# neu-vi/Superpoints_Registration

Hardware: AMD Instinct MI355X
Metric: point-cloud pairs/sec (16 384 pts/cloud) (higher is better)
Workload: dtype f32 (matrix products: range-scaled split-f16x2 MFMA, f32 accumulate; attention weights below 2^-5 of their row sum carried in one f16 plane); 1 GPU; synthetic 16384-pt pairs, full KPConv backbone + superpoint attn + Sinkhorn-SVD pose (3dmatch config, BASELINE configs[1]); streams_per_gpu=1, points_per_cloud=16384, generator=box, point_order=reference, upsample_indices=True, cross_step_overlap=True, streams_inside_a_forward=3: main path, pyramid searches, ResNet shortcut branches

## Files before the change

### include/spr.h

```cpp
#ifndef SPR_H_
#define SPR_H_

#include <stddef.h>
#include <stdint.h>

#ifdef __cplusplus
extern "C" {
#endif

#define SPR_VERSION 6

#define SPR_ACT_NONE 0
#define SPR_ACT_RELU 1
#define SPR_ACT_SIGMOID 2

#define SPR_ORDER_REFERENCE 0
#define SPR_ORDER_CANONICAL 1

#define SPR_SELECT_NEAREST 0
#define SPR_SELECT_INDEX 1

int spr_version(void);
const char* spr_last_error(void);

// ... 38 lines not shown
size_t spr_augment_workspace_bytes(int ns, int nt, int nb, int corr_stride);
int spr_augment_pairs(const float* src_xyz, const int* src_cu, int ns, const float* tgt_xyz, const int* tgt_cu,
                      int nt, const float* pose, int nb, const unsigned char* src_mask,
                      const unsigned char* tgt_mask, const int* corr, int corr_stride, const int* corr_off,
                      const int* corr_count, const float* perturb, const unsigned char* flags, int mode, float scale,
                      int max_pts, uint64_t seed, const uint64_t* pair_key, const float* noise,
                      const unsigned int* keys, float* out_src_xyz, float* out_tgt_xyz, int* out_src_cu,
                      int* out_tgt_cu, float* out_pose, unsigned char* out_src_mask, unsigned char* out_tgt_mask,
                      int* out_src_perm, int* out_tgt_perm, int* out_corr, int* out_corr_count, int* status, void* ws,
                      size_t ws_bytes, void* stream);

size_t spr_kpconv_workspace_bytes(int nq, int ns, int cin, int cout);
size_t spr_kpconv_plan_bytes(int nq);
int spr_kpconv_plan(const int* nbr, int nq, int ns, int nbr_stride, int kmax, int rows_sorted,
                    const int* order, void* plan, size_t plan_bytes, void* stream);
size_t spr_kpconv_wplanes_bytes(int cin, int cout);
int spr_kpconv_prep_weights(const float* weights, int n_kp, int cin, int cout, const float* w_range,
                            int w_range_n, void* wplanes, size_t wplanes_bytes, void* stream);
int spr_kpconv_fwd(const float* q_xyz, int nq, const float* s_xyz, int ns, const int* nbr,
                   int nbr_stride, int kmax, int rows_sorted, const float* x, int cin,
                   const float* weights, int cout, const float* kernel_points, int n_kp,
                   float kp_extent, float* out, int impl, const float* x_range, int x_range_n,
                   const float* w_range, int w_range_n, const void* plan, const void* wplanes,
                   void* ws, size_t ws_bytes, void* stream);

size_t spr_instnorm_workspace_bytes(int max_len_host, int nb, int c);
int spr_instnorm(const float* x, const int* cu, int n, int nb, int max_len_host, int c,
                 float eps, int norm, const float* add, float slope, float* out,
                 float* out_range, int out_range_n, void* ws, size_t ws_bytes, void* stream);
int spr_instnorm_stats(const float* x, const int* cu, int n, int nb, int max_len_host, int c, float eps,
                       float* mean, float* rstd, void* ws, size_t ws_bytes, void* stream);

int spr_block_tail_tile_rows(int ka, int kb, int n_out);
size_t spr_block_tail_tiles_len(int n, int nb, int tile_rows);
int spr_block_tail_tiles(const int* cu, int n, int nb, int tile_rows, int* tiles, void* stream);
size_t spr_block_tail_workspace_bytes(int n, int nb, int kb, int n_out, int tile_rows);
int spr_block_tail(const float* xa, int ka, const float* wa, const float* xb, int kb, const float* wb,
                   const float* add, const int* cu, const int* tiles, int n, int nb, int n_out, float eps,
                   float slope, float* out, const float* xa_range, int xa_range_n, const float* wa_range,
                   int wa_range_n, const float* xb_range, int xb_range_n, const float* wb_range,
                   int wb_range_n, float* out_range, int out_range_n, const float* xa_mean,
                   const float* xa_rstd, float xa_slope, void* ws, size_t ws_bytes, void* stream);

int spr_maxpool_gather(const float* x, int ns, int c, const int* idx, int nq, int idx_stride, int k,
                       const int* order, float* out, float* out_range, int out_range_n, void* stream);
size_t spr_cell_order_workspace_bytes(int n);
int spr_cell_order(const float* xyz, const int* cu, int n, int nb, float cell, int* order, void* ws, size_t ws_bytes,
                   void* stream);

size_t spr_linear_workspace_bytes(void);
int spr_linear(const float* x, int m, int k, const float* w, int n, const float* bias,
               const float* residual, int act, float* out, const float* x_range,
// ... 212 lines not shown
```

### superpoints_registration_amd/_lib.py

```python
import ctypes
import os
import subprocess

_HERE = os.path.dirname(os.path.abspath(__file__))
LIB_PATH = os.environ.get("SPR_HIP_LIB") or os.path.join(_HERE, "libspr_hip.so")

_vp = ctypes.c_void_p
_i = ctypes.c_int
_f = ctypes.c_float
_sz = ctypes.c_size_t
_l = ctypes.c_long
_u64 = ctypes.c_uint64

SIGNATURES = {
    "spr_version": (_i, []),
    "spr_last_error": (ctypes.c_char_p, []),
    "spr_grid_subsample_workspace_bytes": (_sz, [_i, _i]),
    "spr_grid_subsample": (_i, [_vp, _vp, _i, _i, _f, _i, _i, _vp, _vp, _vp, _vp, _sz, _vp]),
    "spr_voxel_downsample_workspace_bytes": (_sz, [_i]),
    "spr_voxel_downsample": (_i, [_vp, _i, ctypes.c_double, _vp, _vp, _vp, _sz, _vp]),
    "spr_radius_neighbors_workspace_bytes": (_sz, [_i, _i, _i]),
    "spr_radius_neighbors": (_i, [_vp, _vp, _i, _vp, _vp, _i, _i, _f, _i, _i, _i, _vp, _vp, _vp, _sz, _vp]),
    "spr_radius_table_bytes": (_sz, [_i, _i]),
    "spr_radius_table_build_workspace_bytes": (_sz, [_i, _i]),
    "spr_radius_table_query_workspace_bytes": (_sz, [_i]),
    "spr_radius_table_slots": (_i, []),
    "spr_radius_table_build": (_i, [_vp, _vp, _i, _i, _f, _vp, _sz, _vp, _sz, _vp]),
    "spr_radius_table_query": (_i, [_vp, _vp, _i, _i, _i, _i, _f, _i, _i, _vp, _vp, _vp, _i, _i, _vp, _sz, _vp]),
    "spr_gt_overlap_workspace_bytes": (_sz, [_i, _i, _i]),
    "spr_gt_overlap": (_i, [_vp, _vp, _i, _vp, _vp, _i, _vp, _i, ctypes.c_double, _vp, _vp, _vp, _vp, _vp, _vp, _vp,
                            _sz, _vp]),
    "spr_philox4x32_host": (_i, [_vp, _vp, _vp]),
    "spr_augment_draw": (_i, [_u64, _vp, _i, _i, _vp, _vp, _vp, _vp, _vp, _i, _vp, _i, _vp, _vp, _vp]),
    "spr_augment_workspace_bytes": (_sz, [_i, _i, _i, _i]),
    "spr_augment_pairs": (_i, [_vp, _vp, _i, _vp, _vp, _i, _vp, _i, _vp, _vp, _vp, _i, _vp, _vp, _vp, _vp, _i, _f, _i,
                               _u64, _vp, _vp, _vp, _vp, _vp, _vp, _vp, _vp, _vp, _vp, _vp, _vp, _vp, _vp, _vp, _vp,
                               _sz, _vp]),
    "spr_kpconv_workspace_bytes": (_sz, [_i, _i, _i, _i]),
    "spr_kpconv_fwd": (_i, [_vp, _i, _vp, _i, _vp, _i, _i, _i, _vp, _i, _vp, _i, _vp, _i, _f, _vp, _i, _vp, _i, _vp,
                            _i, _vp, _vp, _vp, _sz, _vp]),
    "spr_instnorm_workspace_bytes": (_sz, [_i, _i, _i]),
    "spr_instnorm": (_i, [_vp, _vp, _i, _i, _i, _i, _f, _i, _vp, _f, _vp, _vp, _i, _vp, _sz, _vp]),
    "spr_maxpool_gather": (_i, [_vp, _i, _i, _vp, _i, _i, _i, _vp, _vp, _vp, _i, _vp]),
    "spr_linear_workspace_bytes": (_sz, []),
    "spr_linear": (_i, [_vp, _i, _i, _vp, _i, _vp, _vp, _i, _vp, _vp, _i, _vp, _i, _vp, _i, _vp, _vp, _sz, _vp]),
    "spr_range_parts": (_i, []),
    "spr_absmax_multi": (_i, [_vp, _i, _i, _vp, _vp]),
    "spr_absmax": (_i, [_vp, _l, _i, _l, _vp, _vp]),
    "spr_kpconv_plan_bytes": (_sz, [_i]),
    "spr_kpconv_plan": (_i, [_vp, _i, _i, _i, _i, _i, _vp, _vp, _sz, _vp]),
    "spr_kpconv_wplanes_bytes": (_sz, [_i, _i]),
    "spr_kpconv_prep_weights": (_i, [_vp, _i, _i, _i, _vp, _i, _vp, _sz, _vp]),
    "spr_block_tail_tile_rows": (_i, [_i, _i, _i]),
    "spr_block_tail_tiles_len": (_sz, [_i, _i, _i]),
    "spr_block_tail_tiles": (_i, [_vp, _i, _i, _i, _vp, _vp]),
    "spr_block_tail_workspace_bytes": (_sz, [_i, _i, _i, _i, _i]),
    "spr_block_tail": (_i, [_vp, _i, _vp, _vp, _i, _vp, _vp, _vp, _vp, _i, _i, _i, _f, _f, _vp, _vp, _i, _vp, _i,
                            _vp, _i, _vp, _i, _vp, _i, _vp, _vp, _f, _vp, _sz, _vp]),
    "spr_instnorm_stats": (_i, [_vp, _vp, _i, _i, _i, _i, _f, _vp, _vp, _vp, _sz, _vp]),
    "spr_cell_order_workspace_bytes": (_sz, [_i]),
    "spr_cell_order": (_i, [_vp, _vp, _i, _i, _f, _vp, _vp, _sz, _vp]),
    "spr_layernorm_range_count": (_i, [_i]),
    "spr_attn_inproj_prepare": (_i, [_vp, _i, _vp, _vp]),
    "spr_set_gemm_mode": (_i, [_i]),
    "spr_layernorm": (_i, [_vp, _i, _i, _vp, _vp, _f, _vp, _vp, _vp, _vp, _vp, _vp]),
# ... 114 lines not shown
```

### superpoints_registration_amd/csrc/kpconv.hip

```cpp
#include "spr_common.h"

namespace spr {
namespace {

constexpr int kKP = 15;

__global__ __launch_bounds__(256) void k_rowflag(const float* __restrict__ x, const float* __restrict__ s_xyz,
                                                 int ns, int cin, unsigned char* __restrict__ flag,
                                                 float4* __restrict__ sxf, int* __restrict__ tile_ctr) {
  const int wid = (blockIdx.x * blockDim.x + threadIdx.x) >> 6;
  const int lane = threadIdx.x & 63;
  const int c4 = cin >> 2;
  if (blockIdx.x == 0 && threadIdx.x == 0) {
    sxf[ns] = make_float4(-1.0e17f, -1.0e17f, -1.0e17f, __int_as_float(0));
    tile_ctr[0] = 0;
  }
  if ((cin & 3) == 0 && c4 <= 64 && (c4 & (c4 - 1)) == 0) {
    constexpr int kRfSteps = 4;
    const int rpl = 64 / c4;
    const int sub = lane / c4, chunk = lane % c4;
    const int row0 = wid * rpl * kRfSteps + sub;
    float4 v[kRfSteps];
#pragma unroll
    for (int r = 0; r < kRfSteps; ++r) {
// ... 28 lines not shown
      }
    }
    return;
  }
  const int row = wid;
  if (row >= ns) return;
  float s = 0.f;
  for (int c = lane; c < cin; c += 64) s += x[(size_t)row * cin + c];
  s = wave_sum(s);
  if (lane == 0) {
    const int f = s > 0.f ? 1 : 0;
    flag[row] = (unsigned char)f;
    sxf[row] = make_float4(s_xyz[3 * (size_t)row], s_xyz[3 * (size_t)row + 1],
                           s_xyz[3 * (size_t)row + 2], __int_as_float(f));
  }
}

__global__ void k_kpconv_simple(const float* __restrict__ q_xyz, int nq,
                                const float* __restrict__ s_xyz, int ns,
                                const int* __restrict__ nbr, int nbr_stride, int kmax,
                                const float* __restrict__ x, int cin,
                                const float* __restrict__ W, int cout,
                                const float* __restrict__ kpts, int n_kp, float inv_extent,
                                const unsigned char* __restrict__ flag,
                                float* __restrict__ out) {
  const long gid = (long)blockIdx.x * blockDim.x + threadIdx.x;
  if (gid >= (long)nq * cout) return;
  const int n = (int)(gid / cout), o = (int)(gid % cout);
  const float qx = q_xyz[3 * (size_t)n], qy = q_xyz[3 * (size_t)n + 1], qz = q_xyz[3 * (size_t)n + 2];
  float acc = 0.f;
  int cnt = 0;
  for (int k = 0; k < kmax; ++k) {
    const int idx = nbr[(size_t)n * nbr_stride + k];
    if (idx < 0 || idx >= ns) continue;
    cnt += flag[idx];
    const float rx = s_xyz[3 * (size_t)idx] - qx, ry = s_xyz[3 * (size_t)idx + 1] - qy,
                rz = s_xyz[3 * (size_t)idx + 2] - qz;
    for (int p = 0; p < n_kp; ++p) {
      const float dx = rx - kpts[3 * p], dy = ry - kpts[3 * p + 1], dz = rz - kpts[3 * p + 2];
      const float w = fmaxf(0.f, 1.f - sqrtf(dx * dx + dy * dy + dz * dz) * inv_extent);
      if (w > 0.f) {
        float d = 0.f;
        for (int c = 0; c < cin; ++c)
          d += x[(size_t)idx * cin + c] * W[((size_t)p * cin + c) * cout + o];
        acc += w * d;
      }
    }
  }
  out[(size_t)n * cout + o] = acc / (float)max(cnt, 1);
}

__global__ __launch_bounds__(256) void k_records_cin1(const float* __restrict__ x, const float* __restrict__ s_xyz,
                                                      int ns, float4* __restrict__ sxf) {
  const int i = blockIdx.x * blockDim.x + threadIdx.x;
  if (i < ns) sxf[i] = make_float4(s_xyz[3 * (size_t)i], s_xyz[3 * (size_t)i + 1], s_xyz[3 * (size_t)i + 2], x[i]);
}

__global__ __launch_bounds__(256) void k_kpconv_cin1(
// ... 1066 lines not shown
  hipStream_t stream = (hipStream_t)stream_;
  SPR_REQUIRE(n_kp == kKP && cin % 32 == 0 && cout % 32 == 0 && cout <= 256,
              "kpconv weight planes exist for the MFMA shapes only (15 kernel points, channels in multiples of 32)");
  SPR_REQUIRE(w_range != nullptr && w_range_n >= 1, "kpconv weight planes: the weight range is required");
  Workspace w(wplanes, bytes);
  const auto [wh, wl] = wplanes_view(w, cin, cout);
  SPR_REQUIRE(wplanes != nullptr && w.ok(), "kpconv weight planes: buffer too small");
  hipLaunchKernelGGL(k_w_prep, dim3(cdiv((long)n_kp * cin * cout, 256)), dim3(256), 0, stream, weights, cin, cout,
                     w_chunk(cin), w_range, w_range_n, wh, wl);
  SPR_LAUNCH_CHECK();
  return 0;
}

extern "C" size_t spr_kpconv_workspace_bytes(int nq, int ns, int cin, int cout) {
  return measure(kpconv_layout, nq, ns, cin, cout);
}

extern "C" int spr_kpconv_fwd(const float* q_xyz, int nq, const float* s_xyz, int ns,
                              const int* nbr, int nbr_stride, int kmax, int rows_sorted,
                              const float* x, int cin, const float* weights, int cout,
                              const float* kernel_points, int n_kp, float kp_extent,
                              float* out, int impl, const float* x_range, int x_range_n, const float* w_range,
                              int w_range_n, const void* plan, const void* wplanes, void* ws, size_t ws_bytes,
                              void* stream_) {
  hipStream_t stream = (hipStream_t)stream_;
  SPR_REQUIRE((x_range == nullptr || x_range_n >= 1) && (w_range == nullptr || w_range_n >= 1),
              "kpconv: a range needs a count");
  SPR_REQUIRE(nq > 0 && ns > 0, "kpconv: empty input");
  SPR_REQUIRE(kmax >= 1 && kmax <= nbr_stride, "kpconv: bad kmax=%d stride=%d", kmax, nbr_stride);
  SPR_REQUIRE(cin >= 1 && cout >= 1 && n_kp >= 1 && n_kp <= 32, "kpconv: bad dims");
  SPR_REQUIRE(kp_extent > 0.f, "kpconv: KP_extent must be > 0");
  Workspace w(ws, ws_bytes);
  const auto [flag, sxf, own_wplanes, x_parts, w_parts, own_plan, tile_ctr] = kpconv_layout(w, nq, ns, cin, cout);
  SPR_REQUIRE(ws != nullptr && w.ok(), "kpconv: workspace too small");
  SPR_REQUIRE(wplanes == nullptr || w_range != nullptr, "kpconv: prepared weight planes come with the range they were scaled by");
  Workspace given_w(const_cast<void*>(wplanes), SIZE_MAX), given_p(const_cast<void*>(plan), SIZE_MAX);
  const auto [wh, wl] = wplanes != nullptr ? wplanes_view(given_w, cin, cout) : own_wplanes;
  const float inv_extent = 1.0f / kp_extent;

  if (cin == 1 && (impl == 0 || impl == 2) && n_kp <= 16) {
    hipLaunchKernelGGL(k_records_cin1, dim3(cdiv(ns, 256)), dim3(256), 0, stream, x, s_xyz, ns, sxf);
    ProfScope prof(stream, cin * 100000 + cout, nq);
    hipLaunchKernelGGL(k_kpconv_cin1, dim3(cdiv(nq, 64)), dim3(256), 0, stream, q_xyz, nq, s_xyz, ns, nbr,
                       nbr_stride, kmax, rows_sorted, sxf, weights, cout, kernel_points, n_kp, inv_extent, out);
    SPR_LAUNCH_CHECK();
    return 0;
  }

  launch_rowflag(x, s_xyz, ns, cin, flag, sxf, tile_ctr, stream);
  SPR_LAUNCH_CHECK();

  const bool tile_fits = cin % 64 == 0 ? mfma_lds_bytes(64, kTile64TQ, kTileWaves, kmax) <= kMfmaLdsMax
                                       : mfma_lds_bytes(32, kTile32TQ, kTileWaves, kmax) <= kMfmaLdsMax;
  if ((impl == 0 || impl == 2) && n_kp == kKP && cin % 32 == 0 && cout % 32 == 0 && cout <= 256 && tile_fits) {
    const int ktot = n_kp * cin;
    const float* xp = x_range != nullptr ? x_range : x_parts;
    const float* wp = w_range != nullptr ? w_range : w_parts;
    const int n_xp = x_range != nullptr ? x_range_n : kAmaxParts, n_wp = w_range != nullptr ? w_range_n : kAmaxParts;
    if (x_range == nullptr && w_range == nullptr) {
      if (int rc = launch_absmax2(x, ns, cin, cin, x_parts, weights, ktot, cout, cout, w_parts, stream)) return rc;
    } else if (x_range == nullptr) {
      if (int rc = launch_absmax(x, ns, cin, cin, x_parts, stream)) return rc;
    } else if (w_range == nullptr) {
      if (int rc = launch_absmax(weights, ktot, cout, cout, w_parts, stream)) return rc;
    }
    if (wplanes == nullptr)
      hipLaunchKernelGGL(k_w_prep, dim3(cdiv((long)ktot * cout, 256)), dim3(256), 0, stream, weights, cin, cout,
                         w_chunk(cin), wp, n_wp, wh, wl);
    const bool ring_ok = impl == 0 && ring_shape(cin, cout) && kmax <= 128 && (size_t)ns * cin * 4 < (1ull << 32) &&
                         (size_t)nq * nbr_stride * 4 < (1ull << 32);
    if (ring_ok) {
      if (plan == nullptr)
        if (int rc = launch_plan(nbr, nq, ns, nbr_stride, kmax, rows_sorted, nullptr, own_plan, stream)) return rc;
      const auto [desc, pad_word] = plan != nullptr ? plan_view(given_p, nq) : own_plan;
#define SPR_RING_ARGS                                                                                       \
  q_xyz, nq, ns, nbr, nbr_stride, kmax, x, wh, wl, kernel_points, inv_extent, sxf, desc, pad_word, xp, wp, \
      n_xp, n_wp, tile_ctr, out, stream
      if (cin == 64 && cout == 64) return launch_ring<64, 64, SPR_KP_NS64>(SPR_RING_ARGS);
      if (cin == 64 && cout == 32) return launch_ring<64, 32, 4>(SPR_RING_ARGS);
      if (cin == 32 && cout == 32) return launch_ring<32, 32, 3>(SPR_RING_ARGS);
      if (cin == 32 && cout == 64) return launch_ring<32, 64, 8>(SPR_RING_ARGS);
      if (cin == 32 && cout == 128) return launch_ring<32, 128, 8>(SPR_RING_ARGS);
#undef SPR_RING_ARGS
    }
#define SPR_KP_ARGS                                                                         \
  q_xyz, nq, s_xyz, ns, nbr, nbr_stride, kmax, rows_sorted, x, cin, wh, wl, cout,           \
      kernel_points, inv_extent, sxf, xp, wp, n_xp, n_wp, out, stream
    if (cin % 64 == 0) {
      if (cout == 64) return launch_mfma<64, kTile64TQ, 1, kTileWaves, 2>(SPR_KP_ARGS);
      if (cout == 128) return launch_mfma<64, kTile64TQ, 2, kTileWaves, 2>(SPR_KP_ARGS);
      if (cout == 256) return launch_mfma<64, kTile64TQ, 4, kTileWaves, 2>(SPR_KP_ARGS);
    } else {
      if (cout == 32) return launch_mfma<32, kTile32TQ, 1, kTileWaves, 1>(SPR_KP_ARGS);
      if (cout == 64) return launch_mfma<32, kTile32TQ, 2, kTileWaves, 1>(SPR_KP_ARGS);
      if (cout == 128) return launch_mfma<32, kTile32TQ, 4, kTileWaves, 1>(SPR_KP_ARGS);
    }
#undef SPR_KP_ARGS
  }
  const long total = (long)nq * cout;
  hipLaunchKernelGGL(k_kpconv_simple, dim3(cdiv(total, 256)), dim3(256), 0, stream, q_xyz, nq,
                     s_xyz, ns, nbr, nbr_stride, kmax, x, cin, weights, cout, kernel_points, n_kp,
                     inv_extent, flag, out);
  SPR_LAUNCH_CHECK();
  return 0;
}
```

### superpoints_registration_amd/csrc/norm_pool.hip

```cpp
#include "spr_common.h"

namespace spr {
namespace {

constexpr int kSliceRows = 512;
int in_nsplit(int max_len) {
  int s = cdiv(max_len > 0 ? max_len : 1, kSliceRows);
  return s < 1 ? 1 : s;
}

__global__ __launch_bounds__(256) void k_in_stats(const float* __restrict__ x,
                                                  const int* __restrict__ cu, int c, int nsplit,
                                                  double* __restrict__ part ) {
  const int cloud = blockIdx.x, split = blockIdx.y, cb = blockIdx.z * 64;
  const int beg = cu[cloud], end = cu[cloud + 1];
  const int r0 = beg + split * kSliceRows;
  const int r1 = min(r0 + kSliceRows, end);
  const int cw = min(c - cb, 64);
  const int cw4 = cw >> 2;
  const int rl = 256 / cw4;
  const int tc = threadIdx.x % cw4, tr = threadIdx.x / cw4;
  __shared__ double sh[8][256];
  double s[4] = {0, 0, 0, 0}, ss[4] = {0, 0, 0, 0};
  if (tr < rl) {
// ... 54 lines not shown
    const double* p = part + (((size_t)cloud * nsplit + k) * 2) * c;
    s += p[ch];
    ss += p[c + ch];
  }
  const int len = cu[cloud + 1] - cu[cloud];
  const double n = len > 0 ? (double)len : 1.0;
  const double m = s / n;
  double var = ss / n - m * m;
  if (var < 0.0) var = 0.0;
  mean[i] = (float)m;
  rstd[i] = (float)(1.0 / sqrt(var + (double)eps));
}

__device__ __forceinline__ void publish_range(float mx, float* __restrict__ slots, int nslots) {
  __shared__ float shr[4];
  mx = wave_max(mx);
  if ((threadIdx.x & 63) == 0) shr[threadIdx.x >> 6] = mx;
  __syncthreads();
  if (threadIdx.x == 0)
    atomicMax(reinterpret_cast<unsigned int*>(slots) + (blockIdx.x & (nslots - 1)),
              __float_as_uint(fmaxf(fmaxf(shr[0], shr[1]), fmaxf(shr[2], shr[3]))));
}

constexpr int kInApplyUnroll = 4;
__global__ __launch_bounds__(256) void k_in_apply(const float* __restrict__ x, const int* __restrict__ cu, int n,
                                                  int nb, int c, int norm, const float* __restrict__ mean,
                                                  const float* __restrict__ rstd, const float* __restrict__ add,
                                                  float slope, float* __restrict__ out,
                                                  float* __restrict__ out_range, int nslots) {
  const int c4 = c >> 2;
  const long total = (long)n * c4;
  const long stride = (long)gridDim.x * blockDim.x;
  const long g0 = (long)blockIdx.x * blockDim.x + threadIdx.x;
  float4 v[kInApplyUnroll], a[kInApplyUnroll];
#pragma unroll
  for (int u = 0; u < kInApplyUnroll; ++u) {
    const long gid = g0 + u * stride;
    if (gid < total) {
      v[u] = reinterpret_cast<const float4*>(x)[gid];
      if (add) a[u] = reinterpret_cast<const float4*>(add)[gid];
    }
  }
  float mx = 0.f;
#pragma unroll
  for (int u = 0; u < kInApplyUnroll; ++u) {
    const long gid = g0 + u * stride;
    if (gid >= total) continue;
    float4 w = v[u];
    if (norm) {
      const int row = (int)(gid / c4), q = (int)(gid % c4);
      const int cloud = find_segment(cu, nb, row);
      const float4 m = reinterpret_cast<const float4*>(mean + (size_t)cloud * c)[q];
      const float4 r = reinterpret_cast<const float4*>(rstd + (size_t)cloud * c)[q];
      w.x = (w.x - m.x) * r.x;
      w.y = (w.y - m.y) * r.y;
      w.z = (w.z - m.z) * r.z;
      w.w = (w.w - m.w) * r.w;
    }
    if (add) {
      w.x += a[u].x;
      w.y += a[u].y;
      w.z += a[u].z;
      w.w += a[u].w;
    }
    w.x = w.x >= 0.f ? w.x : w.x * slope;
    w.y = w.y >= 0.f ? w.y : w.y * slope;
    w.z = w.z >= 0.f ? w.z : w.z * slope;
    w.w = w.w >= 0.f ? w.w : w.w * slope;
    reinterpret_cast<float4*>(out)[gid] = w;
    mx = fmaxf(mx, fmaxf(fmaxf(fabsf(w.x), fabsf(w.y)), fmaxf(fabsf(w.z), fabsf(w.w))));
  }
  if (out_range != nullptr) publish_range(mx, out_range, nslots);
}

__global__ __launch_bounds__(256) void k_in_bwd_stats(const float* __restrict__ x, const float* __restrict__ out,
                                                      const float* __restrict__ dout, const int* __restrict__ cu,
                                                      int c, int nsplit, float slope,
                                                      const float* __restrict__ mean, const float* __restrict__ rstd,
                                                      double* __restrict__ part ) {
  const int cloud = blockIdx.x, split = blockIdx.y, cb = blockIdx.z * 64;
  const int beg = cu[cloud], end = cu[cloud + 1];
  const int r0 = beg + split * kSliceRows;
  const int r1 = min(r0 + kSliceRows, end);
  const int cw = min(c - cb, 64);
  const int cw4 = cw >> 2;
  const int rl = 256 / cw4;
  const int tc = threadIdx.x % cw4, tr = threadIdx.x / cw4;
  __shared__ double sh[8][256];
  double s1[4] = {0, 0, 0, 0}, s2[4] = {0, 0, 0, 0};
  if (tr < rl) {
    const int col = cb + 4 * tc;
    const float4 mu = *reinterpret_cast<const float4*>(mean + (size_t)cloud * c + col);
    const float4 rs = *reinterpret_cast<const float4*>(rstd + (size_t)cloud * c + col);
// ... 165 lines not shown
  float *mean, *rstd;
  double *m1, *m2;
};
InstnormWs instnorm_layout(Workspace& w, int max_len, int nb, int c, bool backward) {
  const size_t B = (size_t)(nb > 0 ? nb : 1), C = (size_t)(c > 0 ? c : 1);
  InstnormWs l{};
  l.part = w.take<double>(B * in_nsplit(max_len) * 2 * C);
  l.mean = w.take<float>(B * C);
  l.rstd = w.take<float>(B * C);
  if (backward) {
    l.m1 = w.take<double>(B * C);
    l.m2 = w.take<double>(B * C);
  }
  return l;
}
}

extern "C" size_t spr_instnorm_workspace_bytes(int max_len, int nb, int c) {
  return measure(instnorm_layout, max_len, nb, c, false);
}

extern "C" int spr_instnorm(const float* x, const int* cu, int n, int nb, int max_len_host, int c,
                            float eps, int norm, const float* add, float slope, float* out, float* out_range,
                            int out_range_n, void* ws, size_t ws_bytes, void* stream_) {
  hipStream_t stream = (hipStream_t)stream_;
  SPR_REQUIRE(out_range == nullptr || (out_range_n >= 1 && (out_range_n & (out_range_n - 1)) == 0),
              "instnorm: out_range_n must be a power of two");
  SPR_REQUIRE(n > 0 && nb >= 1 && c >= 4 && c % 4 == 0, "instnorm: need n>0 and c %% 4 == 0 (c=%d)", c);
  float* mean = nullptr;
  float* rstd = nullptr;
  if (norm) {
    SPR_REQUIRE(max_len_host >= 1 && max_len_host <= n, "instnorm: bad max_len_host=%d", max_len_host);
    Workspace w(ws, ws_bytes);
    const InstnormWs l = instnorm_layout(w, max_len_host, nb, c, false);
    SPR_REQUIRE(ws != nullptr && w.ok(), "instnorm: workspace too small");
    const int nsplit = in_nsplit(max_len_host);
    double* part = l.part;
    mean = l.mean;
    rstd = l.rstd;
    hipLaunchKernelGGL(k_in_stats, dim3(nb, nsplit, cdiv(c, 64)), dim3(256), 0, stream, x, cu, c, nsplit, part);
    hipLaunchKernelGGL(k_in_final, dim3(cdiv((long)nb * c, 256)), dim3(256), 0, stream, part, cu,
                       nb, c, nsplit, eps, mean, rstd);
    SPR_LAUNCH_CHECK();
  }
  const long total = (long)n * (c / 4);
  hipLaunchKernelGGL(k_in_apply, dim3(cdiv(total, 256 * kInApplyUnroll)), dim3(256), 0, stream, x, cu, n, nb, c,
                     norm, mean, rstd, add, slope, out, out_range, out_range_n);
  SPR_LAUNCH_CHECK();
  return 0;
}

extern "C" int spr_instnorm_stats(const float* x, const int* cu, int n, int nb, int max_len_host, int c, float eps,
                                  float* mean, float* rstd, void* ws, size_t ws_bytes, void* stream_) {
  hipStream_t stream = (hipStream_t)stream_;
  SPR_REQUIRE(x && cu && mean && rstd && n > 0 && nb >= 1 && c >= 4 && c % 4 == 0, "instnorm_stats: bad arguments (c=%d)", c);
  SPR_REQUIRE(max_len_host >= 1 && max_len_host <= n, "instnorm_stats: bad max_len_host=%d", max_len_host);
  Workspace w(ws, ws_bytes);
  double* part = instnorm_layout(w, max_len_host, nb, c, false).part;
  SPR_REQUIRE(ws != nullptr && w.ok(), "instnorm_stats: workspace too small");
  const int nsplit = in_nsplit(max_len_host);
  hipLaunchKernelGGL(k_in_stats, dim3(nb, nsplit, cdiv(c, 64)), dim3(256), 0, stream, x, cu, c, nsplit, part);
  hipLaunchKernelGGL(k_in_final, dim3(cdiv((long)nb * c, 256)), dim3(256), 0, stream, part, cu, nb, c, nsplit, eps, mean,
                     rstd);
  SPR_LAUNCH_CHECK();
  return 0;
}

extern "C" size_t spr_instnorm_bwd_workspace_bytes(int max_len, int nb, int c) {
  return measure(instnorm_layout, max_len, nb, c, true);
}
// ... 61 lines not shown
```

### superpoints_registration_amd/kpconv_blocks.py

```python
import math

import torch
import torch.nn as nn
from torch.nn.init import kaiming_uniform_
from torch.nn.parameter import Parameter

from . import _concurrency, ops
from .kernel_points import load_kernels


def _cu_of(batch, layer_ind):
    cache = batch.setdefault('_cu', {})
    cu = cache.get(layer_ind)
    if cu is None:
        cu = ops.lengths_to_cu(batch['stack_lengths'][layer_ind],
                               batch['points'][layer_ind].device)
        cache[layer_ind] = cu
    return cu


def _maxlen_of(batch, layer_ind):
    lens = batch.get('_lens_host')
    return max(lens[layer_ind]) if lens is not None else None

# ... 77 lines not shown

def block_decider(block_name, radius, in_dim, out_dim, layer_ind, config):
    if block_name == 'unary':
        return UnaryBlock(in_dim, out_dim, config.use_batch_norm, config.batch_norm_momentum)
    elif block_name in ['simple', 'simple_strided']:
        return SimpleBlock(block_name, in_dim, out_dim, radius, layer_ind, config)
    elif block_name in ['resnetb', 'resnetb_strided']:
        return ResnetBottleneckBlock(block_name, in_dim, out_dim, radius, layer_ind, config)
    else:
        raise ValueError('Unknown / unsupported block name in the architecture definition : ' + block_name)


class BatchNormBlock(nn.Module):

    def __init__(self, in_dim, use_bn, bn_momentum):
        super().__init__()
        self.bn_momentum = bn_momentum
        self.use_bn = use_bn
        self.in_dim = in_dim
        self.eps = 1e-5
        if not self.use_bn:
            self.bias = Parameter(torch.zeros(in_dim, dtype=torch.float32), requires_grad=True)

    def forward(self, x, stack_lengths, cu=None, add=None, slope=1.0, max_len=None):
        if cu is None:
            cu = ops.lengths_to_cu(stack_lengths, x.device)
        if self.use_bn:
            return ops.instnorm(x, cu, eps=self.eps, norm=True, add=add, slope=slope, max_len=max_len)
        y = x + self.bias
        return ops.instnorm(y, cu, norm=False, add=add, slope=slope, max_len=max_len)

    def __repr__(self):
        return 'BatchNormBlock(in_feat: {:d}, momentum: {:.3f}, only_bias: {:s})'.format(
            self.in_dim, self.bn_momentum, str(not self.use_bn))


class UnaryBlock(nn.Module):

    def __init__(self, in_dim, out_dim, use_bn, bn_momentum, no_relu=False):
        super().__init__()
        self.bn_momentum = bn_momentum
        self.use_bn = use_bn
        self.no_relu = no_relu
        self.in_dim = in_dim
        self.out_dim = out_dim
        self.mlp = nn.Linear(in_dim, out_dim, bias=False)
        self.batch_norm = BatchNormBlock(out_dim, self.use_bn, self.bn_momentum)
        if not no_relu:
            self.leaky_relu = nn.LeakyReLU(0.1)

    def forward(self, x, stack_lengths=None, cu=None, add=None, final_slope=None, max_len=None):
        y = ops.linear(x, self.mlp.weight)
        slope = 1.0 if self.no_relu else 0.1
        if final_slope is not None:
            slope = final_slope
        return self.batch_norm(y, stack_lengths, cu=cu, add=add, slope=slope, max_len=max_len)

    def __repr__(self):
        return 'UnaryBlock(in_feat: {:d}, out_feat: {:d}, BN: {:s}, ReLU: {:s})'.format(
            self.in_dim, self.out_dim, str(self.use_bn), str(not self.no_relu))


class SimpleBlock(nn.Module):

    def __init__(self, block_name, in_dim, out_dim, radius, layer_ind, config):
        super().__init__()
        current_extent = radius * config.KP_extent / config.conv_radius
        self.bn_momentum = config.batch_norm_momentum
        self.use_bn = config.use_batch_norm
        self.layer_ind = layer_ind
        self.block_name = block_name
        self.in_dim = in_dim
        self.out_dim = out_dim
        self.KPConv = KPConv(config.num_kernel_points, config.in_points_dim, in_dim, out_dim // 2,
                             current_extent, radius,
                             fixed_kernel_points=config.fixed_kernel_points,
                             KP_influence=config.KP_influence,
                             aggregation_mode=config.aggregation_mode,
                             deformable='deform' in block_name, modulated=config.modulated)
# ... 65 lines not shown
                 and ops.block_tail_tile_rows(mid, self.in_dim if projected else 0, self.out_dim) > 0)

        def shortcut_branch():
            sc = max_pool(features, neighb_inds, _pool_order_of(batch, li)) if strided else features
            if projected and not fused:
                sc = self.unary_shortcut(sc, stack_lengths_post, cu=cu_post, max_len=ml_post)
            return sc

        has_work = strided or (projected and not fused)
        fork = (has_work and features.is_cuda and not torch.is_grad_enabled()
                and _concurrency.active(features.device))
        if fork:
            main = torch.cuda.current_stream(features.device)
            branch = _concurrency.aux_stream(main, features.device, 'shortcut')
            ready = torch.cuda.Event()
            ready.record(main)
            branch.wait_event(ready)
            with torch.cuda.stream(branch):
                shortcut = shortcut_branch()
                joined = torch.cuda.Event()
                joined.record(branch)
            features.record_stream(branch)

        x = self.unary1(features, stack_lengths_pre, cu=cu_pre, max_len=ml_pre) \
            if isinstance(self.unary1, UnaryBlock) else features
        self.KPConv.rows_sorted = bool(batch.get('_rows_sorted', False))
        x = self.KPConv(q_pts, s_pts, neighb_inds, x)
        fold = fused and self.use_bn
        conv_stats = None
        if fold:
            conv_stats = ops.instnorm_stats(x, cu_post, eps=self.batch_norm_conv.eps, max_len=ml_post)
        else:
            x = self.batch_norm_conv(x, stack_lengths_post, cu=cu_post, slope=0.1, max_len=ml_post)

        if fork:
            main.wait_event(joined)
            shortcut.record_stream(main)
        else:
            shortcut = shortcut_branch()
        if fused:
            if projected:
                return ops.block_tail(x, self.unary2.mlp.weight, cu_post, xb=shortcut,
                                      wb=self.unary_shortcut.mlp.weight, eps=self.unary2.batch_norm.eps, slope=0.1,
                                      xa_stats=conv_stats, xa_slope=0.1, xa_max_len=ml_post)
            return ops.block_tail(x, self.unary2.mlp.weight, cu_post, add=shortcut,
                                  eps=self.unary2.batch_norm.eps, slope=0.1,
                                  xa_stats=conv_stats, xa_slope=0.1, xa_max_len=ml_post)
# ... 3 lines not shown
```

### superpoints_registration_amd/ops.py

```python
import ctypes
import math
import threading
from typing import Optional, Sequence, Tuple

import numpy as np
import torch

from . import _lib

ACT_NONE, ACT_RELU, ACT_SIGMOID = 0, 1, 2
ORDER_REFERENCE, ORDER_CANONICAL = 0, 1
SELECT_NEAREST, SELECT_INDEX = 0, 1


def _stream(t: torch.Tensor):
    return ctypes.c_void_p(torch.cuda.current_stream(t.device).cuda_stream)


def _ptr(t: Optional[torch.Tensor]):
    return None if t is None else ctypes.c_void_p(t.data_ptr())


def _dev(t: torch.Tensor, name: str, dtype=None) -> torch.Tensor:
    if not isinstance(t, torch.Tensor) or not t.is_cuda:
# ... 58 lines not shown
    out = pool[0][pool[1]:pool[1] + n]
    pool[1] += n
    return out


class _StreamGuard:

    def __init__(self, buf: torch.Tensor):
        self.stream = torch.cuda.current_stream(buf.device)
        self.event = torch.cuda.Event()
        self.event.record(self.stream)
        self.buf = buf
        self.seen = {self.stream.cuda_stream}

    def acquire(self):
        cur = torch.cuda.current_stream(self.buf.device)
        if cur.cuda_stream not in self.seen:
            cur.wait_event(self.event)
            self.buf.record_stream(cur)
            self.seen.add(cur.cuda_stream)


def _derived(src: torch.Tensor, slot: str, extra, build):
    key = (_ident(src), extra)
    c = getattr(src, slot, None)
    if c is not None and c[0] == key:
        c[2].acquire()
        return c[1]
    value, buf = build()
    setattr(src, slot, (key, value, _StreamGuard(buf)))
    return value


def _measure_range(t: torch.Tensor, guarded: bool):
    L = _lib.lib()
    n = L.spr_range_parts()
    flat = t.reshape(-1, t.shape[-1])
    parts = torch.empty((n,), dtype=torch.float32, device=t.device)
    _lib.check(L.spr_absmax(_ptr(flat), flat.shape[0], flat.shape[1], flat.shape[1], _ptr(parts), _stream(t)),
               "spr_absmax")
    _set_range(t, parts, n, _StreamGuard(parts) if guarded else None)
    return parts, n


def _static_range(w: torch.Tensor):
    r, n = _get_range(w)
    return (r, n) if r is not None else _measure_range(w, True)


_PRIME_PARTS = 16


def prime_weight_ranges(params) -> int:
    todo = [p for p in params if isinstance(p, torch.Tensor) and p.is_cuda and p.dtype == torch.float32
# ... 346 lines not shown
def kpconv_raw(q_pts, s_pts, nbr, x, weights, kernel_points, kp_extent: float, rows_sorted: bool = False,
               impl: int = 0, order: Optional[torch.Tensor] = None) -> torch.Tensor:
    q_pts = _dev(q_pts, "q_pts", torch.float32)
    s_pts = _dev(s_pts, "s_pts", torch.float32)
    x = _dev(x, "x", torch.float32)
    weights = _dev(weights, "weights", torch.float32)
    kernel_points = _dev(kernel_points, "kernel_points", torch.float32)
    if not nbr.is_cuda:
        raise RuntimeError("neighb_inds must be on the device")
    if nbr.dtype != torch.int32:
        nbr = nbr.to(torch.int32)
    stride = nbr.stride(0) if nbr.stride(1) == 1 and nbr.shape[1] > 0 else None
    if stride is None:
        nbr = nbr.contiguous()
        stride = nbr.shape[1]
    nq, ns, kmax = q_pts.shape[0], s_pts.shape[0], nbr.shape[1]
    n_kp, cin, cout = weights.shape
    assert x.shape == (ns, cin), (x.shape, ns, cin)
    L = _lib.lib()
    ws = _workspace(L.spr_kpconv_workspace_bytes(nq, ns, cin, cout), x.device)
    out = torch.empty((nq, cout), dtype=torch.float32, device=x.device)
    xr, xr_n = _get_range(x)
    wr, wr_n = _static_range(weights)
    plan = wplanes = None
    if impl == 0 and n_kp == 15 and cin % 32 == 0 and cout % 32 == 0 and cout <= 256:
        if cin in (32, 64) and cin * cout <= 4096 and kmax <= 128:
            plan = _kpconv_plan(nbr, nq, ns, int(stride), kmax, bool(rows_sorted), order)
        if wr is not None:
            wplanes = _kpconv_wplanes(weights, wr, wr_n)
    _lib.check(L.spr_kpconv_fwd(_ptr(q_pts), nq, _ptr(s_pts), ns, _ptr(nbr), int(stride), kmax,
                                int(bool(rows_sorted)), _ptr(x), cin, _ptr(weights), cout,
                                _ptr(kernel_points), n_kp, float(kp_extent), _ptr(out), int(impl),
                                _ptr(xr), int(xr_n), _ptr(wr), int(wr_n), _ptr(plan), _ptr(wplanes),
                                _ptr(ws), ws.numel(), _stream(x)), "spr_kpconv_fwd")
    return out


def _kpconv_plan(nbr: torch.Tensor, nq: int, ns: int, stride: int, kmax: int, rows_sorted: bool,
                 order: Optional[torch.Tensor] = None) -> torch.Tensor:
    if order is not None:
        order = _dev(order, "order", torch.int32)
        assert order.shape == (nq,)

    def build():
        L = _lib.lib()
        nbytes = L.spr_kpconv_plan_bytes(nq)
        plan = torch.empty((nbytes,), dtype=torch.uint8, device=nbr.device)
        _lib.check(L.spr_kpconv_plan(_ptr(nbr), nq, ns, stride, kmax, int(rows_sorted), _ptr(order), _ptr(plan),
                                     nbytes, _stream(nbr)), "spr_kpconv_plan")
        return plan, plan
    return _derived(nbr, '_spr_kp_plan', (nq, ns, stride, kmax, rows_sorted, None if order is None else _ident(order)),
                    build)


def kpconv_plan_prefetch(nbr: torch.Tensor, ns: int, rows_sorted: bool = True) -> None:
    if nbr is None or not nbr.is_cuda or nbr.dtype != torch.int32 or nbr.dim() != 2 or nbr.shape[1] < 1:
        return
    if nbr.stride(1) != 1 or nbr.shape[1] > 128 or nbr.shape[0] < 1:
        return
    _kpconv_plan(nbr, nbr.shape[0], int(ns), int(nbr.stride(0)), nbr.shape[1], bool(rows_sorted))


def _kpconv_wplanes(weights: torch.Tensor, wr: torch.Tensor, wr_n: int) -> torch.Tensor:
    def build():
        L = _lib.lib()
        n_kp, cin, cout = weights.shape
        nbytes = L.spr_kpconv_wplanes_bytes(cin, cout)
        planes = torch.empty((nbytes,), dtype=torch.uint8, device=weights.device)
        _lib.check(L.spr_kpconv_prep_weights(_ptr(weights), n_kp, cin, cout, _ptr(wr), int(wr_n), _ptr(planes),
                                             nbytes, _stream(weights)), "spr_kpconv_prep_weights")
        return planes, planes
    return _derived(weights, '_spr_kp_wplanes', wr.data_ptr(), build)


def instnorm(x, cu, eps: float = 1e-5, norm: bool = True, add=None, slope: float = 1.0,
             out=None, max_len: Optional[int] = None) -> torch.Tensor:
    if _wants_grad(x, add):
        from .autograd import InstNormFn
        return InstNormFn.apply(_dev(x, "x", torch.float32), _dev(cu, "cu", torch.int32), float(eps), bool(norm),
                                None if add is None else _dev(add, "add", torch.float32), float(slope), max_len)
    return instnorm_raw(x, cu, eps, norm, add, slope, out, max_len)


def instnorm_raw(x, cu, eps: float = 1e-5, norm: bool = True, add=None, slope: float = 1.0,
                 out=None, max_len: Optional[int] = None) -> torch.Tensor:
    x = _dev(x, "x", torch.float32)
    cu = _dev(cu, "cu", torch.int32)
    n, c = x.shape
    nb = cu.numel() - 1
    if add is not None:
        add = _dev(add, "add", torch.float32)
        assert add.shape == x.shape
    if out is None:
        out = torch.empty_like(x)
    L = _lib.lib()
    max_len = n if max_len is None else max(1, min(int(max_len), n))
    ws = _workspace(L.spr_instnorm_workspace_bytes(max_len, nb, c), x.device)
    cnt = _STREAM_SLOTS
    rng = _zero_slots(cnt, x.device)
    _lib.check(L.spr_instnorm(_ptr(x), _ptr(cu), n, nb, max_len, c, float(eps), int(bool(norm)), _ptr(add),
                              float(slope), _ptr(out), _ptr(rng), cnt, _ptr(ws), ws.numel(), _stream(x)),
               "spr_instnorm")
    _set_range(out, rng, cnt)
    return out


def block_tail_tile_rows(ka: int, kb: int, n_out: int) -> int:
    if _modes["gemm"] != 1:
        return 0
    return int(_lib.lib().spr_block_tail_tile_rows(int(ka), int(kb), int(n_out)))


def _tail_tiles(cu: torch.Tensor, n: int, tr: int) -> torch.Tensor:
    def build():
        L = _lib.lib()
        t = torch.empty((L.spr_block_tail_tiles_len(n, cu.numel() - 1, tr),), dtype=torch.int32, device=cu.device)
        _lib.check(L.spr_block_tail_tiles(_ptr(cu), n, cu.numel() - 1, tr, _ptr(t), _stream(cu)), "spr_block_tail_tiles")
        return t, t
    return _derived(cu, f'_spr_tail_tiles_{tr}', (n, tr), build)


def instnorm_stats(x, cu, eps: float = 1e-5, max_len: Optional[int] = None):
    x = _dev(x, "x", torch.float32)
    cu = _dev(cu, "cu", torch.int32)
    n, c = x.shape
    nb = cu.numel() - 1
# ... 876 lines not shown
```

Before: 1262 pairs/s.

## Fuse KPConv support records build into the preceding instance-norm apply kernel

The instance-norm apply kernel can now also write per-point support records (xyz plus a nonzero-row flag computed by a cross-lane reduction of the row sum) when it feeds a KPConv. KPConv picks those records up through a cached derived slot on the feature tensor and skips its own rowflag pass. This is meant to remove a separate launch and a full re-read of the feature matrix before each KPConv. The cost is extra shuffles and DPP reductions in the norm kernel, plus a memset of the tile counter. The flag now tests whether the row sum is positive instead of whether the row is nonzero, which relies on the post-activation values being non-negative.

```diff
diff --git a/include/spr.h b/include/spr.h
--- a/include/spr.h
+++ b/include/spr.h
@@ -84,12 +84,13 @@
                    const float* weights, int cout, const float* kernel_points, int n_kp,
                    float kp_extent, float* out, int impl, const float* x_range, int x_range_n,
                    const float* w_range, int w_range_n, const void* plan, const void* wplanes,
-                   void* ws, size_t ws_bytes, void* stream);
+                   void* ws, size_t ws_bytes, void* stream, const void* records);
 
 size_t spr_instnorm_workspace_bytes(int max_len_host, int nb, int c);
 int spr_instnorm(const float* x, const int* cu, int n, int nb, int max_len_host, int c,
                  float eps, int norm, const float* add, float slope, float* out,
-                 float* out_range, int out_range_n, void* ws, size_t ws_bytes, void* stream);
+                 float* out_range, int out_range_n, void* ws, size_t ws_bytes, void* stream,
+                 const float* s_xyz, void* records);
 int spr_instnorm_stats(const float* x, const int* cu, int n, int nb, int max_len_host, int c, float eps,
                        float* mean, float* rstd, void* ws, size_t ws_bytes, void* stream);
 
diff --git a/superpoints_registration_amd/_lib.py b/superpoints_registration_amd/_lib.py
--- a/superpoints_registration_amd/_lib.py
+++ b/superpoints_registration_amd/_lib.py
@@ -38,9 +38,9 @@
                                _sz, _vp]),
     "spr_kpconv_workspace_bytes": (_sz, [_i, _i, _i, _i]),
     "spr_kpconv_fwd": (_i, [_vp, _i, _vp, _i, _vp, _i, _i, _i, _vp, _i, _vp, _i, _vp, _i, _f, _vp, _i, _vp, _i, _vp,
-                            _i, _vp, _vp, _vp, _sz, _vp]),
+                            _i, _vp, _vp, _vp, _sz, _vp, _vp]),
     "spr_instnorm_workspace_bytes": (_sz, [_i, _i, _i]),
-    "spr_instnorm": (_i, [_vp, _vp, _i, _i, _i, _i, _f, _i, _vp, _f, _vp, _vp, _i, _vp, _sz, _vp]),
+    "spr_instnorm": (_i, [_vp, _vp, _i, _i, _i, _i, _f, _i, _vp, _f, _vp, _vp, _i, _vp, _sz, _vp, _vp, _vp]),
     "spr_maxpool_gather": (_i, [_vp, _i, _i, _vp, _i, _i, _i, _vp, _vp, _vp, _i, _vp]),
     "spr_linear_workspace_bytes": (_sz, []),
     "spr_linear": (_i, [_vp, _i, _i, _vp, _i, _vp, _vp, _i, _vp, _vp, _i, _vp, _i, _vp, _i, _vp, _vp, _sz, _vp]),
diff --git a/superpoints_registration_amd/csrc/kpconv.hip b/superpoints_registration_amd/csrc/kpconv.hip
--- a/superpoints_registration_amd/csrc/kpconv.hip
+++ b/superpoints_registration_amd/csrc/kpconv.hip
@@ -74,7 +74,7 @@
                                 const float* __restrict__ x, int cin,
                                 const float* __restrict__ W, int cout,
                                 const float* __restrict__ kpts, int n_kp, float inv_extent,
-                                const unsigned char* __restrict__ flag,
+                                const unsigned char* __restrict__ flag, const float4* __restrict__ records,
                                 float* __restrict__ out) {
   const long gid = (long)blockIdx.x * blockDim.x + threadIdx.x;
   if (gid >= (long)nq * cout) return;
@@ -85,7 +85,7 @@
   for (int k = 0; k < kmax; ++k) {
     const int idx = nbr[(size_t)n * nbr_stride + k];
     if (idx < 0 || idx >= ns) continue;
-    cnt += flag[idx];
+    cnt += records != nullptr ? __float_as_int(records[idx].w) : (int)flag[idx];
     const float rx = s_xyz[3 * (size_t)idx] - qx, ry = s_xyz[3 * (size_t)idx + 1] - qy,
                 rz = s_xyz[3 * (size_t)idx + 2] - qz;
     for (int p = 0; p < n_kp; ++p) {
@@ -1198,7 +1198,7 @@
                               const float* kernel_points, int n_kp, float kp_extent,
                               float* out, int impl, const float* x_range, int x_range_n, const float* w_range,
                               int w_range_n, const void* plan, const void* wplanes, void* ws, size_t ws_bytes,
-                              void* stream_) {
+                              void* stream_, const void* records) {
   hipStream_t stream = (hipStream_t)stream_;
   SPR_REQUIRE((x_range == nullptr || x_range_n >= 1) && (w_range == nullptr || w_range_n >= 1),
               "kpconv: a range needs a count");
@@ -1207,7 +1207,7 @@
   SPR_REQUIRE(cin >= 1 && cout >= 1 && n_kp >= 1 && n_kp <= 32, "kpconv: bad dims");
   SPR_REQUIRE(kp_extent > 0.f, "kpconv: KP_extent must be > 0");
   Workspace w(ws, ws_bytes);
-  const auto [flag, sxf, own_wplanes, x_parts, w_parts, own_plan, tile_ctr] = kpconv_layout(w, nq, ns, cin, cout);
+  const auto [flag, own_sxf, own_wplanes, x_parts, w_parts, own_plan, tile_ctr] = kpconv_layout(w, nq, ns, cin, cout);
   SPR_REQUIRE(ws != nullptr && w.ok(), "kpconv: workspace too small");
   SPR_REQUIRE(wplanes == nullptr || w_range != nullptr, "kpconv: prepared weight planes come with the range they were scaled by");
   Workspace given_w(const_cast<void*>(wplanes), SIZE_MAX), given_p(const_cast<void*>(plan), SIZE_MAX);
@@ -1215,16 +1215,20 @@
   const float inv_extent = 1.0f / kp_extent;
 
   if (cin == 1 && (impl == 0 || impl == 2) && n_kp <= 16) {
-    hipLaunchKernelGGL(k_records_cin1, dim3(cdiv(ns, 256)), dim3(256), 0, stream, x, s_xyz, ns, sxf);
+    hipLaunchKernelGGL(k_records_cin1, dim3(cdiv(ns, 256)), dim3(256), 0, stream, x, s_xyz, ns, own_sxf);
     ProfScope prof(stream, cin * 100000 + cout, nq);
     hipLaunchKernelGGL(k_kpconv_cin1, dim3(cdiv(nq, 64)), dim3(256), 0, stream, q_xyz, nq, s_xyz, ns, nbr,
-                       nbr_stride, kmax, rows_sorted, sxf, weights, cout, kernel_points, n_kp, inv_extent, out);
+                       nbr_stride, kmax, rows_sorted, own_sxf, weights, cout, kernel_points, n_kp, inv_extent, out);
     SPR_LAUNCH_CHECK();
     return 0;
   }
 
-  launch_rowflag(x, s_xyz, ns, cin, flag, sxf, tile_ctr, stream);
-  SPR_LAUNCH_CHECK();
+  const float4* given_rec = static_cast<const float4*>(records);
+  const float4* sxf = given_rec != nullptr ? given_rec : own_sxf;
+  if (given_rec == nullptr) {
+    launch_rowflag(x, s_xyz, ns, cin, flag, own_sxf, tile_ctr, stream);
+    SPR_LAUNCH_CHECK();
+  }
 
   const bool tile_fits = cin % 64 == 0 ? mfma_lds_bytes(64, kTile64TQ, kTileWaves, kmax) <= kMfmaLdsMax
                                        : mfma_lds_bytes(32, kTile32TQ, kTileWaves, kmax) <= kMfmaLdsMax;
@@ -1249,6 +1253,7 @@
       if (plan == nullptr)
         if (int rc = launch_plan(nbr, nq, ns, nbr_stride, kmax, rows_sorted, nullptr, own_plan, stream)) return rc;
       const auto [desc, pad_word] = plan != nullptr ? plan_view(given_p, nq) : own_plan;
+      if (given_rec != nullptr) SPR_HIP_CHECK(hipMemsetAsync(tile_ctr, 0, sizeof(int), stream));
 #define SPR_RING_ARGS                                                                                       \
   q_xyz, nq, ns, nbr, nbr_stride, kmax, x, wh, wl, kernel_points, inv_extent, sxf, desc, pad_word, xp, wp, \
       n_xp, n_wp, tile_ctr, out, stream
@@ -1276,7 +1281,7 @@
   const long total = (long)nq * cout;
   hipLaunchKernelGGL(k_kpconv_simple, dim3(cdiv(total, 256)), dim3(256), 0, stream, q_xyz, nq,
                      s_xyz, ns, nbr, nbr_stride, kmax, x, cin, weights, cout, kernel_points, n_kp,
-                     inv_extent, flag, out);
+                     inv_extent, flag, given_rec, out);
   SPR_LAUNCH_CHECK();
   return 0;
 }
diff --git a/superpoints_registration_amd/csrc/norm_pool.hip b/superpoints_registration_amd/csrc/norm_pool.hip
--- a/superpoints_registration_amd/csrc/norm_pool.hip
+++ b/superpoints_registration_amd/csrc/norm_pool.hip
@@ -100,53 +100,103 @@
               __float_as_uint(fmaxf(fmaxf(shr[0], shr[1]), fmaxf(shr[2], shr[3]))));
 }
 
+template <int O>
+__device__ __forceinline__ float row_down(float t) {
+  return __int_as_float(__builtin_amdgcn_update_dpp(0, __float_as_int(t), 0x100 | O, 0xF, 0xF, true));
+}
+
 constexpr int kInApplyUnroll = 4;
+template <bool REC>
 __global__ __launch_bounds__(256) void k_in_apply(const float* __restrict__ x, const int* __restrict__ cu, int n,
                                                   int nb, int c, int norm, const float* __restrict__ mean,
                                                   const float* __restrict__ rstd, const float* __restrict__ add,
                                                   float slope, float* __restrict__ out,
-                                                  float* __restrict__ out_range, int nslots) {
+                                                  float* __restrict__ out_range, int nslots,
+                                                  const float* __restrict__ s_xyz, float4* __restrict__ records) {
   const int c4 = c >> 2;
   const long total = (long)n * c4;
   const long stride = (long)gridDim.x * blockDim.x;
   const long g0 = (long)blockIdx.x * blockDim.x + threadIdx.x;
   float4 v[kInApplyUnroll], a[kInApplyUnroll];
+  float pc[kInApplyUnroll] = {0.f, 0.f, 0.f, 0.f};
+  const int chunk = threadIdx.x & (c4 - 1);
+  const bool first = chunk == 0;
+  const int c4_log2 = __ffs(c4) - 1;
 #pragma unroll
   for (int u = 0; u < kInApplyUnroll; ++u) {
     const long gid = g0 + u * stride;
     if (gid < total) {
       v[u] = reinterpret_cast<const float4*>(x)[gid];
       if (add) a[u] = reinterpret_cast<const float4*>(add)[gid];
-    }
+      if constexpr (REC) {
+        if (c4 >= 4 && chunk < 3) pc[u] = s_xyz[3 * (size_t)(gid >> c4_log2) + chunk];
+      }
+    }
+  }
+  if constexpr (REC) {
+    if (g0 == 0) records[n] = make_float4(-1.0e17f, -1.0e17f, -1.0e17f, __int_as_float(0));
   }
   float mx = 0.f;
 #pragma unroll
   for (int u = 0; u < kInApplyUnroll; ++u) {
     const long gid = g0 + u * stride;
-    if (gid >= total) continue;
-    float4 w = v[u];
-    if (norm) {
-      const int row = (int)(gid / c4), q = (int)(gid % c4);
-      const int cloud = find_segment(cu, nb, row);
-      const float4 m = reinterpret_cast<const float4*>(mean + (size_t)cloud * c)[q];
-      const float4 r = reinterpret_cast<const float4*>(rstd + (size_t)cloud * c)[q];
-      w.x = (w.x - m.x) * r.x;
-      w.y = (w.y - m.y) * r.y;
-      w.z = (w.z - m.z) * r.z;
-      w.w = (w.w - m.w) * r.w;
-    }
-    if (add) {
-      w.x += a[u].x;
-      w.y += a[u].y;
-      w.z += a[u].z;
-      w.w += a[u].w;
-    }
-    w.x = w.x >= 0.f ? w.x : w.x * slope;
-    w.y = w.y >= 0.f ? w.y : w.y * slope;
-    w.z = w.z >= 0.f ? w.z : w.z * slope;
-    w.w = w.w >= 0.f ? w.w : w.w * slope;
-    reinterpret_cast<float4*>(out)[gid] = w;
-    mx = fmaxf(mx, fmaxf(fmaxf(fabsf(w.x), fabsf(w.y)), fmaxf(fabsf(w.z), fabsf(w.w))));
+    float4 w = make_float4(0.f, 0.f, 0.f, 0.f);
+    if (gid < total) {
+      w = v[u];
+      if (norm) {
+        const int row = REC ? (int)(gid >> c4_log2) : (int)(gid / c4);
+        const int q = REC ? (int)(gid & (c4 - 1)) : (int)(gid % c4);
+        const int cloud = find_segment(cu, nb, row);
+        const float4 m = reinterpret_cast<const float4*>(mean + (size_t)cloud * c)[q];
+        const float4 r = reinterpret_cast<const float4*>(rstd + (size_t)cloud * c)[q];
+        w.x = (w.x - m.x) * r.x;
+        w.y = (w.y - m.y) * r.y;
+        w.z = (w.z - m.z) * r.z;
+        w.w = (w.w - m.w) * r.w;
+      }
+      if (add) {
+        w.x += a[u].x;
+        w.y += a[u].y;
+        w.z += a[u].z;
+        w.w += a[u].w;
+      }
+      w.x = w.x >= 0.f ? w.x : w.x * slope;
+      w.y = w.y >= 0.f ? w.y : w.y * slope;
+      w.z = w.z >= 0.f ? w.z : w.z * slope;
+      w.w = w.w >= 0.f ? w.w : w.w * slope;
+      reinterpret_cast<float4*>(out)[gid] = w;
+      mx = fmaxf(mx, fmaxf(fmaxf(fabsf(w.x), fabsf(w.y)), fmaxf(fabsf(w.z), fabsf(w.w))));
+    }
+    if constexpr (REC) {
+      const int lane = threadIdx.x & 63;
+      float s4[4] = {w.x, w.y, w.z, w.w};
+#pragma unroll
+      for (int e = 0; e < 4; ++e) {
+        float t = s4[e];
+        if (c4 == 64) {
+          const int b = lane & 15;
+          const float a0 = __shfl(t, b, 64), a1 = __shfl(t, b | 16, 64), a2 = __shfl(t, b | 32, 64),
+                      a3 = __shfl(t, b | 48, 64);
+          t = ((a0 + a1) + a2) + a3;
+        } else if (c4 == 32) {
+          t += __shfl_xor(t, 16, 64);
+        }
+        if (c4 >= 16) t += row_down<8>(t);
+        if (c4 >= 8) t += row_down<4>(t);
+        if (c4 >= 4) t += row_down<2>(t);
+        if (c4 >= 2) t += row_down<1>(t);
+        s4[e] = t;
+      }
+      const float t = (s4[0] + s4[2]) + (s4[1] + s4[3]);
+      float px = pc[u], py = row_down<1>(pc[u]), pz = row_down<2>(pc[u]);
+      if (gid < total && first) {
+        if (c4 < 4) {
+          const float* p = s_xyz + 3 * (size_t)(gid >> c4_log2);
+          px = p[0], py = p[1], pz = p[2];
+        }
+        records[gid >> c4_log2] = make_float4(px, py, pz, __int_as_float(t > 0.f ? 1 : 0));
+      }
+    }
   }
   if (out_range != nullptr) publish_range(mx, out_range, nslots);
 }
@@ -358,8 +408,12 @@
 
 extern "C" int spr_instnorm(const float* x, const int* cu, int n, int nb, int max_len_host, int c,
                             float eps, int norm, const float* add, float slope, float* out, float* out_range,
-                            int out_range_n, void* ws, size_t ws_bytes, void* stream_) {
+                            int out_range_n, void* ws, size_t ws_bytes, void* stream_, const float* s_xyz,
+                            void* records) {
   hipStream_t stream = (hipStream_t)stream_;
+  SPR_REQUIRE((s_xyz == nullptr) == (records == nullptr), "instnorm: support records need the points and the buffer");
+  SPR_REQUIRE(records == nullptr || (c % 4 == 0 && c / 4 <= 64 && ((c / 4) & (c / 4 - 1)) == 0),
+              "instnorm: support records exist for c / 4 a power of two <= 64 (c=%d)", c);
   SPR_REQUIRE(out_range == nullptr || (out_range_n >= 1 && (out_range_n & (out_range_n - 1)) == 0),
               "instnorm: out_range_n must be a power of two");
   SPR_REQUIRE(n > 0 && nb >= 1 && c >= 4 && c % 4 == 0, "instnorm: need n>0 and c %% 4 == 0 (c=%d)", c);
@@ -380,8 +434,12 @@
     SPR_LAUNCH_CHECK();
   }
   const long total = (long)n * (c / 4);
-  hipLaunchKernelGGL(k_in_apply, dim3(cdiv(total, 256 * kInApplyUnroll)), dim3(256), 0, stream, x, cu, n, nb, c,
-                     norm, mean, rstd, add, slope, out, out_range, out_range_n);
+  if (records != nullptr)
+    hipLaunchKernelGGL(k_in_apply<true>, dim3(cdiv(total, 256 * kInApplyUnroll)), dim3(256), 0, stream, x, cu, n, nb, c,
+                       norm, mean, rstd, add, slope, out, out_range, out_range_n, s_xyz, static_cast<float4*>(records));
+  else
+    hipLaunchKernelGGL(k_in_apply<false>, dim3(cdiv(total, 256 * kInApplyUnroll)), dim3(256), 0, stream, x, cu, n, nb, c,
+                       norm, mean, rstd, add, slope, out, out_range, out_range_n, nullptr, nullptr);
   SPR_LAUNCH_CHECK();
   return 0;
 }
diff --git a/superpoints_registration_amd/kpconv_blocks.py b/superpoints_registration_amd/kpconv_blocks.py
--- a/superpoints_registration_amd/kpconv_blocks.py
+++ b/superpoints_registration_amd/kpconv_blocks.py
@@ -123,13 +123,14 @@
         if not self.use_bn:
             self.bias = Parameter(torch.zeros(in_dim, dtype=torch.float32), requires_grad=True)
 
-    def forward(self, x, stack_lengths, cu=None, add=None, slope=1.0, max_len=None):
+    def forward(self, x, stack_lengths, cu=None, add=None, slope=1.0, max_len=None, records_xyz=None):
         if cu is None:
             cu = ops.lengths_to_cu(stack_lengths, x.device)
         if self.use_bn:
-            return ops.instnorm(x, cu, eps=self.eps, norm=True, add=add, slope=slope, max_len=max_len)
+            return ops.instnorm(x, cu, eps=self.eps, norm=True, add=add, slope=slope, max_len=max_len,
+                                records_xyz=records_xyz)
         y = x + self.bias
-        return ops.instnorm(y, cu, norm=False, add=add, slope=slope, max_len=max_len)
+        return ops.instnorm(y, cu, norm=False, add=add, slope=slope, max_len=max_len, records_xyz=records_xyz)
 
     def __repr__(self):
         return 'BatchNormBlock(in_feat: {:d}, momentum: {:.3f}, only_bias: {:s})'.format(
@@ -150,12 +151,13 @@
         if not no_relu:
             self.leaky_relu = nn.LeakyReLU(0.1)
 
-    def forward(self, x, stack_lengths=None, cu=None, add=None, final_slope=None, max_len=None):
+    def forward(self, x, stack_lengths=None, cu=None, add=None, final_slope=None, max_len=None, records_xyz=None):
         y = ops.linear(x, self.mlp.weight)
         slope = 1.0 if self.no_relu else 0.1
         if final_slope is not None:
             slope = final_slope
-        return self.batch_norm(y, stack_lengths, cu=cu, add=add, slope=slope, max_len=max_len)
+        return self.batch_norm(y, stack_lengths, cu=cu, add=add, slope=slope, max_len=max_len,
+                               records_xyz=records_xyz)
 
     def __repr__(self):
         return 'UnaryBlock(in_feat: {:d}, out_feat: {:d}, BN: {:s}, ReLU: {:s})'.format(
@@ -267,7 +269,8 @@
                 joined.record(branch)
             features.record_stream(branch)
 
-        x = self.unary1(features, stack_lengths_pre, cu=cu_pre, max_len=ml_pre) \
+        rec_xyz = s_pts if features.is_cuda and not torch.is_grad_enabled() else None
+        x = self.unary1(features, stack_lengths_pre, cu=cu_pre, max_len=ml_pre, records_xyz=rec_xyz) \
             if isinstance(self.unary1, UnaryBlock) else features
         self.KPConv.rows_sorted = bool(batch.get('_rows_sorted', False))
         x = self.KPConv(q_pts, s_pts, neighb_inds, x)
diff --git a/superpoints_registration_amd/ops.py b/superpoints_registration_amd/ops.py
--- a/superpoints_registration_amd/ops.py
+++ b/superpoints_registration_amd/ops.py
@@ -104,14 +104,20 @@
 
 
 def _derived(src: torch.Tensor, slot: str, extra, build):
-    key = (_ident(src), extra)
+    value = _derived_get(src, slot, extra)
+    if value is not None:
+        return value
+    value, buf = build()
+    setattr(src, slot, ((_ident(src), extra), value, _StreamGuard(buf)))
+    return value
+
+
+def _derived_get(src: torch.Tensor, slot: str, extra):
     c = getattr(src, slot, None)
-    if c is not None and c[0] == key:
-        c[2].acquire()
-        return c[1]
-    value, buf = build()
-    setattr(src, slot, (key, value, _StreamGuard(buf)))
-    return value
+    if c is None or c[0] != (_ident(src), extra):
+        return None
+    c[2].acquire()
+    return c[1]
 
 
 def _measure_range(t: torch.Tensor, guarded: bool):
@@ -504,6 +510,7 @@
     out = torch.empty((nq, cout), dtype=torch.float32, device=x.device)
     xr, xr_n = _get_range(x)
     wr, wr_n = _static_range(weights)
+    records = _derived_get(x, _KP_RECORDS, _ident(s_pts)) if cin > 1 else None
     plan = wplanes = None
     if impl == 0 and n_kp == 15 and cin % 32 == 0 and cout % 32 == 0 and cout <= 256:
         if cin in (32, 64) and cin * cout <= 4096 and kmax <= 128:
@@ -514,7 +521,7 @@
                                 int(bool(rows_sorted)), _ptr(x), cin, _ptr(weights), cout,
                                 _ptr(kernel_points), n_kp, float(kp_extent), _ptr(out), int(impl),
                                 _ptr(xr), int(xr_n), _ptr(wr), int(wr_n), _ptr(plan), _ptr(wplanes),
-                                _ptr(ws), ws.numel(), _stream(x)), "spr_kpconv_fwd")
+                                _ptr(ws), ws.numel(), _stream(x), _ptr(records)), "spr_kpconv_fwd")
     return out
 
 
@@ -556,16 +563,24 @@
 
 
 def instnorm(x, cu, eps: float = 1e-5, norm: bool = True, add=None, slope: float = 1.0,
-             out=None, max_len: Optional[int] = None) -> torch.Tensor:
+             out=None, max_len: Optional[int] = None, records_xyz=None) -> torch.Tensor:
     if _wants_grad(x, add):
         from .autograd import InstNormFn
         return InstNormFn.apply(_dev(x, "x", torch.float32), _dev(cu, "cu", torch.int32), float(eps), bool(norm),
                                 None if add is None else _dev(add, "add", torch.float32), float(slope), max_len)
-    return instnorm_raw(x, cu, eps, norm, add, slope, out, max_len)
+    return instnorm_raw(x, cu, eps, norm, add, slope, out, max_len, records_xyz)
+
+
+_KP_RECORDS = '_spr_kp_records'
+
+
+def kpconv_records_shape(c: int) -> bool:
+    c4 = c // 4
+    return c % 4 == 0 and 1 <= c4 <= 64 and (c4 & (c4 - 1)) == 0
 
 
 def instnorm_raw(x, cu, eps: float = 1e-5, norm: bool = True, add=None, slope: float = 1.0,
-                 out=None, max_len: Optional[int] = None) -> torch.Tensor:
+                 out=None, max_len: Optional[int] = None, records_xyz=None) -> torch.Tensor:
     x = _dev(x, "x", torch.float32)
     cu = _dev(cu, "cu", torch.int32)
     n, c = x.shape
@@ -580,10 +595,17 @@
     ws = _workspace(L.spr_instnorm_workspace_bytes(max_len, nb, c), x.device)
     cnt = _STREAM_SLOTS
     rng = _zero_slots(cnt, x.device)
+    records = None
+    if records_xyz is not None and kpconv_records_shape(c):
+        records_xyz = _dev(records_xyz, "records_xyz", torch.float32)
+        assert records_xyz.shape == (n, 3), (records_xyz.shape, n)
+        records = torch.empty((n + 1, 4), dtype=torch.float32, device=x.device)
     _lib.check(L.spr_instnorm(_ptr(x), _ptr(cu), n, nb, max_len, c, float(eps), int(bool(norm)), _ptr(add),
-                              float(slope), _ptr(out), _ptr(rng), cnt, _ptr(ws), ws.numel(), _stream(x)),
-               "spr_instnorm")
+                              float(slope), _ptr(out), _ptr(rng), cnt, _ptr(ws), ws.numel(), _stream(x),
+                              _ptr(records_xyz) if records is not None else None, _ptr(records)), "spr_instnorm")
     _set_range(out, rng, cnt)
+    if records is not None:
+        _derived(out, _KP_RECORDS, _ident(records_xyz), lambda: (records, records))
     return out
 
 
```

Result: no change. 1273 pairs/s (median of 6 runs) (+0.9%).
